# Mehooz/vision4leg

Measured on AMD Instinct MI355X. Metric: PPO env-steps/s (encoder+update, sim excluded), higher is better.
Workload: dtype f16; 1 GPU; ppo_locotransformer thin-goal: LocoTransformer S=93 A=6, E=32 envs x T=512, B=1024, 3 opt epochs; net=loco, envs_per_gpu=32, horizon=512, minibatch=1024, opt_epochs=3, parallelism=dp1, includes_rollout_inference=True, logp_old=recorded at action time (target_pf forward skipped; SURVEY 8d declared saving)

## Files before the change

### vision4leg_amd/csrc/gemm.h

```cpp
#pragma once
#include "common.h"

namespace v4l {

struct RowCtx {
  int64_t base;
  int a, b;
  int valid;
};

__device__ __forceinline__ void zero8(float (&v)[8]) {
#pragma unroll
  for (int j = 0; j < 8; ++j) v[j] = 0.f;
}
__device__ __forceinline__ void ld8(const float* p, float (&v)[8]) {
  const float4 x = *reinterpret_cast<const float4*>(p);
  const float4 y = *reinterpret_cast<const float4*>(p + 4);
  v[0] = x.x; v[1] = x.y; v[2] = x.z; v[3] = x.w;
  v[4] = y.x; v[5] = y.y; v[6] = y.z; v[7] = y.w;
}
template <typename H>
__device__ __forceinline__ void ld8(const H* p, float (&v)[8]) {
  static_assert(sizeof(H) == 2, "16-bit operand type");
  typedef typename HVec<H, 4>::type bf16x4;
  const bf16x4 x = *reinterpret_cast<const bf16x4*>(p);
  const bf16x4 y = *reinterpret_cast<const bf16x4*>(p + 4);
#pragma unroll
  for (int j = 0; j < 4; ++j) { v[j] = (float)x[j]; v[4 + j] = (float)y[j]; }
}

template <int W> __device__ __forceinline__ void ldv(const float* p, float (&v)[W]) {
  if constexpr (W == 1) v[0] = p[0];
  else if constexpr (W == 2) { const float2 x = *reinterpret_cast<const float2*>(p); v[0] = x.x; v[1] = x.y; }
  else { const float4 x = *reinterpret_cast<const float4*>(p); v[0] = x.x; v[1] = x.y; v[2] = x.z; v[3] = x.w; }
}
template <int W, typename H> __device__ __forceinline__ void ldv(const H* p, float (&v)[W]) {
  static_assert(sizeof(H) == 2, "16-bit operand type");
  if constexpr (W == 1) v[0] = (float)p[0];
  else {
    typedef typename HVec<H, W>::type bv_t;
    const bv_t x = *reinterpret_cast<const bv_t*>(p);
#pragma unroll
    for (int i = 0; i < W; ++i) v[i] = (float)x[i];
  }
}

__device__ __forceinline__ void keep8(float (&v)[8], bool ok) {
#pragma unroll
  for (int j = 0; j < 8; ++j) v[j] = ok ? v[j] : 0.f;
}

struct ADense {
  const float* p;
  int lda, M, K;
  const int* rowidx;
  int tokmap;
  const float* mask;
  __device__ __forceinline__ RowCtx row(int m) const {
    RowCtx rc;
    rc.valid = m < M;
    rc.a = rc.b = 0;
    int r = m;
    if (tokmap == 1) r = (m >> 4) * 17 + 1 + (m & 15);
    if (rowidx != nullptr) r = rowidx[rc.valid ? m : 0];
    rc.base = (int64_t)r * lda;
    return rc;
  }
  __device__ __forceinline__ void load(const RowCtx& rc, int k0, float (&v)[8]) const {
    const bool ok = rc.valid && k0 < K;
    const int64_t off = ok ? rc.base + k0 : 0;
    ld8(p + off, v);
    if (mask != nullptr) {
      float mk[8];
      ld8(mask + off, mk);
#pragma unroll
      for (int j = 0; j < 8; ++j) v[j] = mk[j] > 0.f ? v[j] : 0.f;
    }
    keep8(v, ok);
  }
  struct RowIt { int m; };
  __device__ __forceinline__ RowIt iter(int m) const { return RowIt{m}; }
  __device__ __forceinline__ int64_t off(const RowIt& it, int& valid) const { return row_off(it.m, valid); }
  __device__ __forceinline__ void next(RowIt& it) const { ++it.m; }
  __device__ __forceinline__ int64_t row_off(int m, int& valid) const { RowCtx rc = row(m); valid = rc.valid; return rc.base; }
  __device__ __forceinline__ int64_t col_off(int k, int& valid) const { valid = k < K; return k; }
  __device__ __forceinline__ float get(int64_t off) const {
    const float v = p[off];
    if (mask == nullptr) return v;
    const float mk = mask[off];
// ... 543 lines not shown

  float* out = slab + (int64_t)bz * Npad * Kpad;
#pragma unroll
  for (int i = 0; i < NT; ++i) {
    const int n = n0 + i * 16 + (lane & 15);
#pragma unroll
    for (int j = 0; j < KT; ++j) {
      const int k4 = k0 + (wave * KT + j) * 16 + (lane >> 4) * 4;
      if (n < Npad && k4 < Kpad)
        *reinterpret_cast<float4*>(out + (int64_t)n * Kpad + k4) = float4{acc[i][j][0], acc[i][j][1], acc[i][j][2], acc[i][j][3]};
    }
  }
  if (do_bias) {
    sBias[wave][lane] = bsum;
    __syncthreads();
    if (tid < BN && n0 + tid < Npad)
      bslab[(int64_t)bz * Npad + n0 + tid] = sBias[0][tid] + sBias[1][tid] + sBias[2][tid] + sBias[3][tid];
  }
}

template <typename T, int BN, int KT, class YL, class XL>
__global__ __launch_bounds__(256) void gemm_tn_kernel(YL yl, XL xl, int M, int m_per_block, float* __restrict__ slab,
                                                      float* __restrict__ bslab, int Npad, int Kpad) {
  tn_body<T, BN, KT, YL, XL>(yl, xl, M, m_per_block, slab, bslab, Npad, Kpad, blockIdx.x, blockIdx.y, blockIdx.z);
}

struct TnProb {
  ADense y, x;
  int M, mpb, Npad, Kpad, gx, gy;
  float* slab;
  float* bslab;
  int64_t blk0;
};
struct ADenseG {
  const V4L_GLOBAL float* p;
  const V4L_GLOBAL int* rowidx;
  const V4L_GLOBAL float* mask;
  int lda, M, K, tokmap;
  __device__ __forceinline__ explicit ADenseG(const ADense& a)
      : p(as_global(a.p)), rowidx(as_global(a.rowidx)), mask(as_global(a.mask)), lda(a.lda), M(a.M), K(a.K), tokmap(a.tokmap) {}
  struct RowIt { int m; };
  __device__ __forceinline__ RowIt iter(int m) const { return RowIt{m}; }
  __device__ __forceinline__ void next(RowIt& it) const { ++it.m; }
  __device__ __forceinline__ int64_t off(const RowIt& it, int& valid) const {
    const int m = it.m;
    valid = m < M;
    int r = m;
    if (tokmap == 1) r = (m >> 4) * 17 + 1 + (m & 15);
    if (a_rowidx()) r = rowidx[valid ? m : 0];
    return (int64_t)r * lda;
  }
  __device__ __forceinline__ bool a_rowidx() const { return rowidx != nullptr; }
  __device__ __forceinline__ int64_t col_off(int k, int& valid) const { valid = k < K; return k; }
  __device__ __forceinline__ float get(int64_t o) const {
    const float v = p[o];
    if (mask == nullptr) return v;
    const float mk = mask[o];
    return mk > 0.f ? v : 0.f;
  }
  template <int W> __device__ __forceinline__ void getv(int64_t o, float (&v)[W]) const {
#pragma unroll
    for (int i = 0; i < W; ++i) v[i] = get(o + i);
  }
};
template <typename T>
__global__ __launch_bounds__(256) void gemm_tn_group_kernel(const TnProb* __restrict__ probs, int np) {
  const TnProb p = probs[find_desc(probs, np, (int64_t)blockIdx.x)];
  const int lb = (int)((int64_t)blockIdx.x - p.blk0);
  const int bx = lb % p.gx, t = lb / p.gx;
  tn_body<T, 64, 1, ADenseG, ADenseG>(ADenseG(p.y), ADenseG(p.x), p.M, p.mpb, p.slab, p.bslab, p.Npad, p.Kpad, bx, t % p.gy,
                                      t / p.gy);
}

struct TnWide {
  const void *y, *x;
  int M, mpb, N, K;
  float *slab, *bslab;
  int blk0, pad;
};
template <typename T> struct Pair;
template <> struct Pair<__bf16> { typedef __attribute__((ext_vector_type(2))) __bf16 type; };
template <> struct Pair<_Float16> { typedef __attribute__((ext_vector_type(2))) _Float16 type; };
template <> struct Pair<float> { typedef __attribute__((ext_vector_type(2))) float type; };
template <typename H>
__device__ __forceinline__ void st8raw(H* dst, const H (&v)[8]) {
  static_assert(sizeof(H) == 2, "16-bit operand type");
  typename Frag<H>::type t;
#pragma unroll
  for (int j = 0; j < 8; ++j) t[j] = v[j];
  *reinterpret_cast<typename Frag<H>::type*>(dst) = t;
}
__device__ __forceinline__ void st8raw(float* dst, const float (&v)[8]) {
  *reinterpret_cast<float4*>(dst) = float4{v[0], v[1], v[2], v[3]};
  *reinterpret_cast<float4*>(dst + 4) = float4{v[4], v[5], v[6], v[7]};
}
template <typename T> struct TnWideLds {
  static constexpr int LD = 64 + (sizeof(T) == 2 ? 8 : 4);
  static constexpr size_t bytes(int N, int K) { return (size_t)(N + K) * LD * sizeof(T) + (size_t)8 * N * 4; }
  static constexpr size_t max_bytes = (size_t)(256 + 64) * LD * sizeof(T) + (size_t)8 * 256 * 4;
};

template <typename T, int N, int K>
__device__ __forceinline__ void tn_wide_body(const TnWide& p, int bz, unsigned char* smem) {
  constexpr int LD = TnWideLds<T>::LD;
  constexpr int NC = N / 64, KC = K / 64;
  constexpr bool SPLIT_N = N > 64;
  static_assert(!SPLIT_N || K == 64, "tn_wide: unsupported shape");
  constexpr int NT_W = SPLIT_N ? N / 64 : 4;
  constexpr int KT_W = SPLIT_N ? 4 : K / 64;
  typedef typename Frag<T>::type frag_t;
  typedef typename Pair<T>::type pair_t;
  T* sY = reinterpret_cast<T*>(smem);
  T* sX = sY + N * LD;
  float* sB = reinterpret_cast<float*>(sX + K * LD);
  const int tid = threadIdx.x, lane = tid & 63, wave = tid >> 6;
  const int half = lane >> 5, cl = (lane & 31) * 2;
  const int mb = bz * p.mpb, me = min(p.M, mb + p.mpb);
  const V4L_GLOBAL T* Y = as_global(reinterpret_cast<const T*>(p.y));
  const V4L_GLOBAL T* X = as_global(reinterpret_cast<const T*>(p.x));
  typedef const V4L_GLOBAL pair_t* gpair_t;
  pair_t yv[NC][8], xv[KC][8];
  float bs[NC][2];
#pragma unroll
  for (int q = 0; q < NC; ++q) bs[q][0] = bs[q][1] = 0.f;
  auto gload = [&](int ms) {
    const int r0 = ms + wave * 16 + half * 8;
#pragma unroll
    for (int j = 0; j < 8; ++j) {
// ... 82 lines not shown
    for (int k = 0; k < 8; ++k) t += sB[k * N + tid];
    as_global(p.bslab)[(int64_t)bz * N + tid] = t;
  }
}

template <typename T>
__global__ __launch_bounds__(256) void gemm_tn_wide_kernel(const TnWide* __restrict__ probs, int np) {
  extern __shared__ __attribute__((aligned(16))) unsigned char tn_wide_smem[];
  int pi = 0;
  for (int i = 1; i < np; ++i) pi = probs[i].blk0 <= (int)blockIdx.x ? i : pi;
  const TnWide p = probs[pi];
  const int bz = (int)blockIdx.x - p.blk0;
  if (p.N == 256 && p.K == 64) tn_wide_body<T, 256, 64>(p, bz, tn_wide_smem);
  else if (p.N == 192 && p.K == 64) tn_wide_body<T, 192, 64>(p, bz, tn_wide_smem);
  else if (p.N == 64 && p.K == 256) tn_wide_body<T, 64, 256>(p, bz, tn_wide_smem);
  else tn_wide_body<T, 64, 64>(p, bz, tn_wide_smem);
}
template <typename T>
__global__ __launch_bounds__(256) void gemm_tn_dense_kernel(const TnWide* __restrict__ wprobs, int nw, int wblocks,
                                                            const TnProb* __restrict__ gprobs, int ng) {
  extern __shared__ __attribute__((aligned(16))) unsigned char tn_wide_smem[];
  if ((int)blockIdx.x < wblocks) {
    int pi = 0;
    for (int i = 1; i < nw; ++i) pi = wprobs[i].blk0 <= (int)blockIdx.x ? i : pi;
    const TnWide p = wprobs[pi];
    const int bz = (int)blockIdx.x - p.blk0;
    if (p.N == 256 && p.K == 64) tn_wide_body<T, 256, 64>(p, bz, tn_wide_smem);
    else if (p.N == 192 && p.K == 64) tn_wide_body<T, 192, 64>(p, bz, tn_wide_smem);
    else if (p.N == 64 && p.K == 256) tn_wide_body<T, 64, 256>(p, bz, tn_wide_smem);
    else tn_wide_body<T, 64, 64>(p, bz, tn_wide_smem);
  } else {
    const int64_t b = (int64_t)blockIdx.x - wblocks;
    const TnProb p = gprobs[find_desc(gprobs, ng, b)];
    const int lb = (int)(b - p.blk0);
    const int bx = lb % p.gx, t = lb / p.gx;
    tn_body<T, 64, 1, ADenseG, ADenseG, true>(ADenseG(p.y), ADenseG(p.x), p.M, p.mpb, p.slab, p.bslab, p.Npad, p.Kpad, bx,
                                              t % p.gy, t / p.gy, tn_wide_smem);
  }
}
static inline bool tn_wide_shape(int N, int K) {
  return (N == 256 && K == 64) || (N == 192 && K == 64) || (N == 64 && K == 256) || (N == 64 && K == 64);
}

constexpr int CONV_BWD_MAX_BLOCKS = 256;

struct RedDesc {
  const float* slab;
  const float* bslab;
  float* dW;
  float* db;
  int nsplit, N, K, Npad, Kpad, Ktorch, Cin, taps;
  int64_t blk0;
  int group, pad_;
};
__global__ __launch_bounds__(256) void wgrad_reduce_kernel(const RedDesc* __restrict__ descs, int nd, float* __restrict__ sq_part,
                                                           int blk_base, float unscale) {
  __shared__ float part[4][64];
  const int64_t bid = (int64_t)blockIdx.x + blk_base;
  const RedDesc d = descs[find_desc(descs, nd, bid)];
  const int o = threadIdx.x & 63, g = threadIdx.x >> 6;
  const int64_t e = (bid - d.blk0) * 64 + o;
  const int64_t nk = (int64_t)d.N * d.K;
  const V4L_GLOBAL float* p = nullptr;
  int64_t stride = 0;
  int n = 0, k = 0;
  if (e < nk) {
    n = (int)(e / d.K); k = (int)(e - (int64_t)n * d.K);
    p = as_global(d.slab) + (int64_t)n * d.Kpad + k;
    stride = (int64_t)d.Npad * d.Kpad;
  } else if (d.db != nullptr && e < nk + d.N) {
// ... 33 lines not shown
```

### vision4leg_amd/csrc/net.h

```cpp
#pragma once
#include <string>
#include <vector>

#include "../../include/v4l_hip.h"
#include "elem.h"
#include "gemm.h"

namespace v4l { struct RowsChain; struct FbLoss; }

namespace v4l {

struct ParamInfo {
  std::string name;
  int ndim;
  int64_t shape[4];
  int64_t numel;
  int64_t goff;
};

struct Lin {
  int w = -1, b = -1;
  int N = 0, K = 0;
  int Np = 0, Kp = 0;
  int64_t pk = 0;
// ... 42 lines not shown
  std::vector<int64_t> deh;
  std::vector<LayerBw> lb;
  std::vector<int64_t> dxl;
  int64_t dhc = 0;
  int64_t dpool = 0, dc3 = 0, dc2 = 0, dc1 = 0;
  std::vector<int64_t> wps_wg, wps_tk;
  int64_t slab = 0;
  int64_t total = 0;
};

enum class LayerFamily {
  NONE,
  WPS_PLAIN,
  WPS_VIS,
  WPS_VIS17,
  WPS_OPT,
  WPS_OPT_VIS,
  BLOCK_STACK,
  BLOCK_PER_LAYER,
  LAYER_BY_LAYER,
};
struct LayerRoute {
  LayerFamily family = LayerFamily::NONE;
  bool heads_in = false;
  bool tail_in = false;
  bool rows17 = false;
  bool fb_allowed = false;
  bool heads_ext_allowed = false;
  bool heads_ext_critic = false;
  bool taps = false;
  bool stack_ok = true;
  bool tok0_in = false;
  int par_wgrad = 2;
  bool wps() const { return family >= LayerFamily::WPS_PLAIN && family <= LayerFamily::WPS_OPT_VIS; }
  bool opt() const { return family == LayerFamily::WPS_OPT || family == LayerFamily::WPS_OPT_VIS; }
  bool block() const { return family == LayerFamily::BLOCK_STACK || family == LayerFamily::BLOCK_PER_LAYER; }
};

}

struct v4l_net {
  v4l_net_cfg cfg;
  int Sp = 0;
  int ntok = v4l::NTOK;
  bool want_acts16 = false;
  const float* acts16_c1 = nullptr;
  bool vis_only() const { return cfg.kind == V4L_NET_CNN_VIS || cfg.kind == V4L_NET_LOCO_VIS; }
  bool is_tf() const { return cfg.kind == V4L_NET_LOCO || cfg.kind == V4L_NET_LOCO_VIS; }
  std::vector<v4l::ParamInfo> params;
  int64_t total_params = 0;
  v4l::Conv conv[3];
  v4l::Lin upconv, proj;
  std::vector<v4l::Lin> enc;
  std::vector<v4l::TLayer> layers;
  v4l::LNp fin_ln;
  v4l::LNp tok_ln, stok_ln;
  std::vector<v4l::Lin> head;
  int logstd = -1;
  int64_t packed_elems = 0;
  std::vector<v4l::PackDesc> packs;
  std::vector<int> pack_param;
  int64_t pack_blocks = 0;
  std::vector<float*> p;
  void* packed = nullptr;
  v4l::PackDesc* d_packs = nullptr;
  v4l::ParamSeg* d_segs = nullptr;
// ... 84 lines not shown
```

### vision4leg_amd/csrc/v4l_hip.hip

```cpp
#include <math.h>
#include <stdarg.h>

#include <algorithm>
#include <type_traits>

#include <dlfcn.h>

#include "net.h"
#include "infer.h"
#include "bwd.h"
#include "wps.h"
#include "wps_fb.h"
#include "rollout_dense.h"
#include "dense_stack.h"
#include "host_step.h"

namespace v4l {

static thread_local char g_err[1024] = "";
static bool sw_on(const char* name) { return getenv(name) != nullptr; }
template <typename T> struct TypeTag { typedef T type; };
#ifdef V4L_DEV_ONLY
template <class F> static inline int by_compute(int compute, F&& f) {
  typedef std::conditional<V4L_DEV_ONLY == V4L_BF16, __bf16, std::conditional<V4L_DEV_ONLY == V4L_F16, _Float16, float>::type>::type T;
// ... 267 lines not shown
    V4L_REQUIRE(net->tnp.size() <= (size_t)v4l_net::MAX_TNP, "internal: too many deferred weight-grads");
    for (TnProb& q : net->tnp) { const int64_t nb = q.blk0; q.blk0 = gb; gb += nb; }
    const size_t bytes = net->tnp.size() * sizeof(TnProb);
    if (net->tnp_cached.size() != net->tnp.size() || memcmp(net->tnp_cached.data(), net->tnp.data(), bytes) != 0) {
      V4L_REQUIRE(!capturing(c.s), "internal: weight-grad geometry changed while capturing a graph");
      V4L_HIP_CHECK(hipStreamSynchronize(c.s));
      V4L_HIP_CHECK(hipMemcpy(net->d_tnp, net->tnp.data(), bytes, hipMemcpyHostToDevice));
      net->tnp_cached = net->tnp;
    }
  }
  if (!net->wide.empty()) {
    V4L_REQUIRE(net->wide.size() <= (size_t)v4l_net::MAX_WIDE, "internal: too many fused-layer weight-grads");
    for (TnWide& q : net->wide) { const int nb = q.blk0; q.blk0 = wb; wb += nb; }
    const size_t bytes = net->wide.size() * sizeof(TnWide);
    if (net->wide_cached.size() != net->wide.size() || memcmp(net->wide_cached.data(), net->wide.data(), bytes) != 0) {
      V4L_REQUIRE(!capturing(c.s), "internal: weight-grad geometry changed while capturing a graph");
      V4L_HIP_CHECK(hipStreamSynchronize(c.s));
      V4L_HIP_CHECK(hipMemcpy(net->d_wide, net->wide.data(), bytes, hipMemcpyHostToDevice));
      net->wide_cached = net->wide;
    }
  }
  constexpr size_t dense_lds = TnWideLds<T>::max_bytes > TnBodyLds<T, 64, 1>::bytes ? TnWideLds<T>::max_bytes : TnBodyLds<T, 64, 1>::bytes;
  V4L_HIP_CHECK(lds_limit<&gemm_tn_wide_kernel<T>>(TnWideLds<T>::max_bytes));
  V4L_HIP_CHECK(lds_limit<&gemm_tn_dense_kernel<T>>(dense_lds));
  if (gb > 0 && wb > 0) {
    g_op = "layer.wgrad";
    V4L_KLAUNCH("gemm_tn_dense", net->wide_flops + net->tnp_flops, dg, gemm_tn_dense_kernel<T>, dim3((unsigned)(wb + gb)), dim3(256),
                dense_lds, dg, (const TnWide*)net->d_wide, (int)net->wide.size(), wb, (const TnProb*)net->d_tnp, (int)net->tnp.size());
    V4L_LAUNCH_CHECK();
    return 0;
  }
  if (gb > 0) {
    g_op = "dense.wgrad";
    V4L_KLAUNCH("gemm_tn_group", net->tnp_flops, dg, gemm_tn_group_kernel<T>, dim3((unsigned)gb), dim3(256), 0, dg,
                (const TnProb*)net->d_tnp, (int)net->tnp.size());
    V4L_LAUNCH_CHECK();
  }
  if (wb > 0) {
    g_op = "layer.wgrad";
    V4L_KLAUNCH("gemm_tn_wide", net->wide_flops, dg, gemm_tn_wide_kernel<T>, dim3((unsigned)wb), dim3(256),
                TnWideLds<T>::max_bytes, dg, (const TnWide*)net->d_wide, (int)net->wide.size());
    V4L_LAUNCH_CHECK();
  }
  return 0;
}
static int wgrad_reduce_prepare(Ctx& c, int64_t (&blocks)[2]) {
  v4l_net* net = c.net;
  std::stable_partition(net->red.begin(), net->red.end(), [](const RedDesc& d) { return d.group == 1; });
  int64_t blk = 0;
  blocks[0] = blocks[1] = 0;
  for (RedDesc& d : net->red) {
    d.blk0 = blk;
    const int64_t nb = cdiv64((int64_t)d.N * d.K + d.N, 64);
    blk += nb;
    blocks[d.group == 1 ? 0 : 1] += nb;
  }
  V4L_REQUIRE(net->red.size() <= (size_t)v4l_net::MAX_RED, "internal: too many weight-grad descriptors");
  const size_t bytes = net->red.size() * sizeof(RedDesc);
  if (net->red_cached.size() != net->red.size() || memcmp(net->red_cached.data(), net->red.data(), bytes) != 0) {
    V4L_REQUIRE(!capturing(c.s), "internal: weight-grad geometry changed while capturing a graph");
    V4L_HIP_CHECK(hipStreamSynchronize(c.s));
    if (c.tn != c.s) V4L_HIP_CHECK(hipStreamSynchronize(c.tn));
    V4L_HIP_CHECK(hipMemcpy(net->d_red, net->red.data(), bytes, hipMemcpyHostToDevice));
    net->red_cached = net->red;
  }
  float* sq = blk <= net->sq_cap() ? net->d_sq : nullptr;
  net->red_blocks = sq != nullptr ? (int)blk : 0;
  net->red_grads = c.grads;
// ... 645 lines not shown
  return 0;
}

int64_t v4l_net::table_bytes() const {
  return (int64_t)(packs.size() * sizeof(PackDesc) + params.size() * sizeof(ParamSeg) + MAX_RED * sizeof(RedDesc) +
                   MAX_TNP * sizeof(TnProb) + MAX_WIDE * sizeof(TnWide) + sq_cap() * sizeof(float) + 1024);
}
static bool dense_stack_shape(const v4l_net* N) {
  const v4l_net_cfg& c = N->cfg;
  if (sw_on("V4L_NO_DENSE_STACK")) return false;
  if (c.n_head_hidden != 2 || c.head_hidden[0] != 256 || c.head_hidden[1] != 256 || c.out_dim > OUT_LD) return false;
  for (int i = 0; i < 3; ++i)
    if (N->head[i].pkf < 0 || N->head[i].pkft < 0) return false;
  if (c.kind == V4L_NET_CNN_VIS) return N->head[0].Kp == 1024 && N->head[0].Rt == 1024;
  if (c.kind != V4L_NET_CNN) return false;
  return c.visual_dim == 256 && c.n_enc_hidden == 2 && c.enc_hidden[0] == 256 && c.enc_hidden[1] == 256 && N->proj.pkf >= 0 &&
         N->proj.pkft >= 0 && N->proj.Kp == 1024 && N->enc[1].pkft >= 0 && N->head[0].Kp == 512;
}
static bool mlp_256(const v4l_net_cfg& c) {
  return c.n_enc_hidden == 2 && c.enc_hidden[0] == 256 && c.enc_hidden[1] == 256 && c.state_dim <= 128;
}
static bool head_256(const v4l_net_cfg& c) { return c.n_head_hidden == 2 && c.head_hidden[0] == 256 && c.head_hidden[1] == 256; }
static bool depth_64(const v4l_net_cfg& c) { return c.in_channels == 4 && c.img_hw == 64; }
bool v4l_net::wps_tail_shape() const {
  return cfg.n_enc_hidden == 2 && cfg.enc_hidden[0] == 256 && cfg.enc_hidden[1] == 256;
}
LayerRoute v4l_net::layer_route(bool whole_pass) const {
  const v4l_net_cfg& c = cfg;
  LayerRoute r;
  r.taps = sw_on("V4L_LAYER_TAPS");
  r.stack_ok = !sw_on("V4L_NO_LAYER_STACK");
  r.tok0_in = sw_on("V4L_WPS_TOK0_IN");
  r.par_wgrad = sw_int("V4L_PAR_WGRAD", 2);
  const bool no_wps = sw_on("V4L_NO_WPS_LAYERS"), vis17 = sw_on("V4L_VIS17"), no_fb = sw_on("V4L_NO_FB");
  const bool head_in = sw_on("V4L_WPS_HEAD_IN"), ext_critic = sw_on("V4L_WPS_HEAD_EXT_CRITIC");
  if (!is_tf()) return r;
  const bool vis = c.kind == V4L_NET_LOCO_VIS, opt = c.token_norm || c.pytorch_encoder;
  const bool heads = head_256(c) && c.out_dim <= OUT_LD;
  const bool wps = c.ff_dim == 256 && c.n_layers == 2 && heads && layers[0].inproj.pkp >= 0 && !no_wps &&
                   (!vis || head[0].pko >= 0);
  const bool around = wps && whole_pass && !c.max_pool && r.stack_ok && !r.taps;
  r.family = LayerFamily::LAYER_BY_LAYER;
  if (vis) {
    if (wps && whole_pass && !opt) r.family = (vis17 || r.taps) ? LayerFamily::WPS_VIS17 : LayerFamily::WPS_VIS;
    else if (around && opt) r.family = LayerFamily::WPS_OPT_VIS;
    r.rows17 = r.wps();
    r.heads_in = r.wps() && !c.pytorch_encoder;
    r.tail_in = r.wps() && !c.token_norm;
    return r;
  }
  const bool plain = !opt && wps_tail_shape();
  if (wps && plain && r.stack_ok) {
    r.family = LayerFamily::WPS_PLAIN;
    r.heads_in = r.tail_in = true;
    r.heads_ext_allowed = !head_in && !r.taps;
    r.heads_ext_critic = r.heads_ext_allowed && ext_critic;
    r.fb_allowed = r.heads_ext_allowed && !c.max_pool && !no_fb && !ext_critic && c.out_dim <= ACT_CAP_NARROW;
  } else if (around && !plain) {
    r.family = LayerFamily::WPS_OPT;
    r.heads_in = !c.pytorch_encoder;
    r.tail_in = !c.token_norm && wps_tail_shape();
  } else if (c.ff_dim == 256 && !opt) {
    r.heads_in = c.n_layers >= 1 && heads && !c.max_pool;
    r.tail_in = c.n_layers >= 1 && wps_tail_shape();
    r.family = (r.heads_in && c.n_layers == 2 && r.stack_ok) ? LayerFamily::BLOCK_STACK : LayerFamily::BLOCK_PER_LAYER;
  }
// ... 589 lines not shown
    float* hand = ws + L.dhc;
    Epi din = mk_epi(hand, cw, cw);
    if ((rc = chain_bwd<T>(cx, head.data(), nh + 1, dense(ws + L.vis, cw, n, cw), hacts, dy, dhhp, &din))) return rc;
    {
      ADense yv = dense(hand, cw, n, c.visual_dim, nullptr, 0, ws + L.vis);
      if ((rc = lin_wgrad<T>(cx, proj, yv, dense(ws + L.c3, 1024, n, 1024), 1024))) return rc;
      Epi ep = mk_epi(ws + L.dc3, 1024, 1024);
      ep.mask = ws + L.c3;
      ep.ldmask = 1024;
      if ((rc = lin_dgrad<T>(cx, proj, yv, ep))) return rc;
    }
    {
      ADense ys = dense(hand + c.visual_dim, cw, n, c.enc_hidden[ne - 1], nullptr, 0, ws + L.vis + c.visual_dim);
      if ((rc = chain_bwd<T>(cx, enc.data(), ne, sin, eacts, ys, dehp, nullptr))) return rc;
    }
    return conv_bwd_and_wgrads();
  }

  if (c.kind == V4L_NET_CNN_VIS) {
    Epi din = mk_epi(ws + L.dc3, 1024, 1024);
    din.mask = ws + L.c3;
    din.ldmask = 1024;
    if ((rc = chain_bwd<T>(cx, head.data(), nh + 1, dense(ws + L.c3, 1024, n, 1024), hacts, dy, dhhp, &din))) return rc;
    return conv_bwd_and_wgrads();
  }

  const bool vis = c.kind == V4L_NET_LOCO_VIS;
  const int pw = vis ? TD : 2 * TD;
  const bool vis_opt = r.family == LayerFamily::WPS_OPT_VIS;
  const int R = n * (vis_opt ? NTOK : ntok);
  auto zero_row0 = [&](float* rows) {
    return hipMemset2DAsync(rows, (size_t)NTOK * TD * sizeof(float), 0, (size_t)TD * sizeof(float), (size_t)n, s);
  };
  if (r.heads_in) {
    if ((rc = lin_wgrad<T>(cx, head[2], dy, dense(hacts[1].p, 256, n, 256), 256))) return rc;
    if ((rc = lin_wgrad<T>(cx, head[1], dense(dhhp[1], 256, n, 256), dense(hacts[0].p, 256, n, 256), 256))) return rc;
    if (r.rows17) rc = lin_wgrad<T>(cx, head[0], dense(dhhp[0], 256, n, 256), dense(ws + L.pooled + TD, 2 * TD, n, TD), TD);
    else rc = lin_wgrad<T>(cx, head[0], dense(dhhp[0], 256, n, 256), dense(ws + L.pooled, 2 * TD, n, 2 * TD), 2 * TD);
    if (rc) return rc;
  } else {
    Epi din = mk_epi(ws + L.dpool, pw, pw);
    if ((rc = chain_bwd<T>(cx, head.data(), nh + 1, dense(ws + L.pooled, pw, n, pw), hacts, dy, dhhp, &din)))
      return rc;
    g_op = "pool";
    float* dlast = c.pytorch_encoder ? ws + L.dxfin : ws + L.dxl[c.n_layers];
    const float* xlast = c.pytorch_encoder ? ws + L.xfin : ws + L.x[c.n_layers];
    if (vis_opt) V4L_HIP_CHECK(zero_row0(dlast));
    if (vis)
      V4L_KLAUNCH("pool_bwd", 0, s, pool_all_bwd_kernel, dim3(n), dim3(64), 0, s, ws + L.dpool, n, ntok, vis_opt ? NTOK : ntok,
                  dlast + (vis_opt ? TD : 0), xlast + (vis_opt ? TD : 0), c.max_pool);
    else
      V4L_KLAUNCH("pool_bwd", 0, s, pool_bwd_kernel, dim3(n), dim3(64), 0, s, ws + L.dpool, n, dlast, xlast, c.max_pool);
    V4L_LAUNCH_CHECK();
    if (c.pytorch_encoder) {
      g_op = "final_ln";
      if ((rc = ln_bwd_launch(cx, std::min(cdiv(R, 16), 128), dlast, ws + L.dxl[c.n_layers], ws + L.xhF, ws + L.rsF, fin_ln, R))) return rc;
    }
  }
  const int lnb = std::min(cdiv(R, 16), 128);
  auto reduce_ln_partials = [&](const TLayer& t, const float* part, int nblk) {
    const int lnp[4] = {t.ln2.g, t.ln2.b, t.ln1.g, t.ln1.b};
    for (int q = 0; q < 4; ++q) {
      RedDesc o;
      memset(&o, 0, sizeof(o));
      o.slab = part + (int64_t)q * nblk * TD;
      o.dW = grads + params[lnp[q]].goff;
      o.nsplit = nblk; o.N = 1; o.K = TD; o.Npad = 1; o.Kpad = TD; o.Ktorch = TD;
      red.push_back(o);
    }
  };
  const bool stacked = r.family == LayerFamily::BLOCK_STACK && r.tail_in;
  if (r.wps()) {
// ... 35 lines not shown
      bt.wpt = base + proj.pkt; bt.wf2t = base + enc[1].pkt;
      bt.s_e1 = eacts[1].p; bt.s_e0 = eacts[0].p; bt.o_dhc = ws + L.dhc; bt.o_de0 = dehp[0];
    }
    WpsTailExtra tx;
    tx.wupt_f = base + upconv.pkpt;
    tx.dpool = ws + L.dpool;
    tx.xlast = c.max_pool ? ws + L.x[c.n_layers] : nullptr;
    tx.dyrows = !r.heads_in ? ws + L.dxl[c.n_layers] : nullptr;
    g_op = "layer";
    const double fl_heads = 2.0 * n * 2 * (16 * 256 + 256 * 256 + 256 * 128) / 2, fl_tok0 = 2.0 * n * (64 * 256 + 256 * 256);
    const double fl = 2 * 4.0 * n * 872576.0 + (head_ext ? 0.0 : 2 * fl_heads) + (tok0_ext ? 0.0 : fl_tok0) + 2.0 * n * 16 * 64 * 64;
#define V4L_WPS_BWD(TAPS_, VIS_, HIN_, TIN_, MODE_)                                                                       \
  do {                                                                                                                    \
    V4L_HIP_CHECK(lds_limit<&wps_layer_bwd_kernel<T, 2, TAPS_, VIS_, HIN_, TIN_, MODE_>>(WpsBwdLds<T>::bytes));            \
    V4L_KLAUNCH("wps_layer_bwd_stack", fl, s, (wps_layer_bwd_kernel<T, 2, TAPS_, VIS_, HIN_, TIN_, MODE_>), dim3(nblk), dim3(256), \
                (WpsBwdLds<T>::bytes), s, d, bh, bt, tx, n);                                                              \
  } while (0)
    const FbLoss* fbl = fb_loss;
    fb_loss = nullptr;
    V4L_REQUIRE(fbl == nullptr || (r.fb_allowed && !head_ext),
                "internal: a fused forward-loss-backward pass was prepared for a net that does not take it");
    const bool m_out = r.opt() && !r.tail_in, m_in = r.opt() && !r.heads_in;
    if (fbl != nullptr) {
      InfLayerStack fst;
      memset(&fst, 0, sizeof(fst));
      fst.nl = 2;
      for (int k = 0; k < 2; ++k)
        fst.l[k].n[0] = inf_layer<T>(this, layers[k], true, k == 0 ? ws + L.x[0] : nullptr);
      InfHeadPair fhd;
      memset(&fhd, 0, sizeof(fhd));
      fhd.n[0] = inf_head<T>(this, L, ws, false);
      FbLoss lo = *fbl;
      lo.dout = ws + L.dout;
      cx.slab_used = (cx.slab_used + 1) & ~(int64_t)1;
      lo.part = reinterpret_cast<double*>(cx.slab + cx.slab_used);
      V4L_REQUIRE((reinterpret_cast<uintptr_t>(lo.part) & 7) == 0, "internal: partial-statistics block not 8-byte aligned");
      cx.slab_used += 2 * (int64_t)nblk * FB_PART;
      V4L_REQUIRE(cx.slab_used <= slab_cap, "internal: weight-grad slab arena overflow");
      const double fl_fb = fl + 2.0 * n * (2 * 872576.0 + 99840.0);
      V4L_HIP_CHECK(lds_limit<&wps_layer_fb_kernel<T, true>>(WpsFbLds<T>::bytes));
      V4L_HIP_CHECK(lds_limit<&wps_layer_fb_kernel<T, false>>(WpsFbLds<T>::bytes));
      if (tok0_ext)
        V4L_KLAUNCH("wps_layer_fb_stack", fl_fb, s, (wps_layer_fb_kernel<T, false>), dim3(nblk), dim3(256), (WpsFbLds<T>::bytes), s, fst,
                    fhd, d, bh, bt, tx, lo, n);
      else
        V4L_KLAUNCH("wps_layer_fb_stack", fl_fb, s, (wps_layer_fb_kernel<T, true>), dim3(nblk), dim3(256), (WpsFbLds<T>::bytes), s, fst,
                    fhd, d, bh, bt, tx, lo, n);
      cx.fb_pending = true;
      cx.fb_args = lo;
      cx.fb_blocks = nblk;
      cx.fb_n = n;
    } else
    switch (r.family) {
      case LayerFamily::WPS_OPT_VIS:
        if (m_out && m_in) V4L_WPS_BWD(false, 2, true, true, 3);
        else if (m_in) V4L_WPS_BWD(false, 2, true, true, 2);
        else V4L_WPS_BWD(false, 2, true, true, 1);
        break;
      case LayerFamily::WPS_OPT:
        if (m_out && m_in) V4L_WPS_BWD(false, false, true, true, 3);
        else if (m_in) V4L_WPS_BWD(false, false, true, true, 2);
        else V4L_WPS_BWD(false, false, true, true, 1);
        break;
      case LayerFamily::WPS_VIS17:
        if (taps) V4L_WPS_BWD(true, true, true, true, 0);
        else V4L_WPS_BWD(false, true, true, true, 0);
// ... 1754 lines not shown
```

### vision4leg_amd/csrc/wps_fb.h

```cpp
#pragma once
#include "wps.h"

#pragma clang fp contract(on)

namespace v4l {

enum { FBP_LP = 0, FBP_LP2, FBP_SUR, FBP_LPMAX, FBP_LPMIN, FBP_RMAX, FBP_RMIN, FBP_SAT, FBP_DL = 8, FBP_VF = 16, FB_PART = 24 };

struct FbLoss {
  int actor;
  const float *ret, *oldv;
  int clipped;
  float clip;
  ActorArgs aa;
  const int* rowidx;
  float inv_n, gscale;
  float* dout;
  double* part;
  float* st;
};

template <typename T> struct WpsFbLds {
  static constexpr bool LDSW = sizeof(T) == 2;
  static constexpr size_t f_b = WpsFwdLds<T>::main_b, b_b = WpsBwdLds<T>::main_b;
  static constexpr size_t main_b = f_b > b_b ? f_b : b_b;
  static constexpr size_t red_b = WpsBwdLds<T>::red_b;
  static constexpr size_t so_b = 16 * 16 * 4;
  static constexpr size_t rec_b = (size_t)WPS_WPB * FB_PART * 8;
  static constexpr size_t bytes = main_b + (size_t)WPS_P_TOTAL * 4 + red_b + so_b + rec_b;
  static_assert(bytes <= 160 * 1024, "one block per CU");
};

__device__ __forceinline__ ActorRow fb_actor_row(const ActorArgs& p, const ActorDims& D, const float (&mu)[8], int slot, float amean,
                                                 float astd) {
  ActorRow o;
  float lp = 0.f;
#pragma unroll
  for (int a = 0; a < 8; ++a) {
    if (a < p.A) {
      const float act = p.acts[(int64_t)slot * p.A + a];
      const float d = act - mu[a];
      const float var = D.sg[a] * D.sg[a];
      lp += -(d * d) / (2.f * var) - D.lsg[a] - HALF_LOG_2PI - 0.f;
      o.z2[a] = d * d / var;
      o.dm[a] = d / var;
    } else {
      o.z2[a] = 0.f; o.dm[a] = 0.f;
    }
  }
  const float lpo = p.logp_old[slot];
  const float ratio = expf(lp - lpo);
  const float an = (p.adv[slot] - amean) / (astd + 1e-5f);
// ... 73 lines not shown
#pragma unroll
    for (int mt = 0; mt < 2; ++mt)
#pragma unroll
      for (int nt = 0; nt < 4; ++nt) xr[mt][nt] = xo[mt][nt];
  }
  float4 mk0[4], mk1[4];
  {
    const InfHead& h = fhd.n[0];
    float* pooled = reinterpret_cast<float*>(smem);
    T* h1 = reinterpret_cast<T*>(pooled + 16 * LF::LDP);
    T* h2 = h1 + 16 * LF::LDF;
    float4 hb0[4], hb1[4];
    float hb2[4];
#pragma unroll
    for (int j = 0; j < 4; ++j) {
      hb0[j] = *reinterpret_cast<const float4*>(h.b0 + nt4[j] * 16 + qr);
      hb1[j] = *reinterpret_cast<const float4*>(h.b1 + nt4[j] * 16 + qr);
      hb2[j] = h.b2[min(qr + j, h.nout - 1)];
    }
    GemmRing<T, 4, 4> ring0 = gemm_prefetch<T, 4, 4>((const T*)h.w0, 128, nt4, lane);
    __syncthreads();
    for (int i = tid; i < 16 * LF::LDP; i += 256) pooled[i] = 0.f;
    __syncthreads();
#pragma unroll
    for (int nt = 0; nt < 4; ++nt) {
      const float4 m = fr == 0 ? xr[1][nt] : xr[0][nt];
      const float4 mv = float4{rowsum16(m.x) * (1.f / 16.f), rowsum16(m.y) * (1.f / 16.f), rowsum16(m.z) * (1.f / 16.f),
                               rowsum16(m.w) * (1.f / 16.f)};
      if (fr == 0 && live) {
        const float4 t0 = xr[0][nt];
        *reinterpret_cast<float4*>(pooled + wave * LF::LDP + nt * 16 + qr) = t0;
        *reinterpret_cast<float4*>(pooled + wave * LF::LDP + TD + nt * 16 + qr) = mv;
        if (h.s_pooled != nullptr) {
          *reinterpret_cast<float4*>(h.s_pooled + (int64_t)smp * 128 + nt * 16 + qr) = t0;
          *reinterpret_cast<float4*>(h.s_pooled + (int64_t)smp * 128 + TD + nt * 16 + qr) = mv;
        }
      }
    }
    __syncthreads();
    f32x4 acc[1][4];
    auto store_h = [&](T* dst, const float4 (&bias)[4], float* save, float4 (&mk)[4]) {
#pragma unroll
      for (int j = 0; j < 4; ++j) {
        const int n4 = nt4[j] * 16 + qr;
        const float4 bb = bias[j];
        const float v0 = fmaxf(acc[0][j][0] + bb.x, 0.f), v1 = fmaxf(acc[0][j][1] + bb.y, 0.f);
        const float v2 = fmaxf(acc[0][j][2] + bb.z, 0.f), v3 = fmaxf(acc[0][j][3] + bb.w, 0.f);
        mk[j] = float4{v0, v1, v2, v3};
        st4(dst + fr * LF::LDF + n4, v0, v1, v2, v3);
        if (fr < ns) st4(save + (int64_t)(s0 + fr) * 256 + n4, v0, v1, v2, v3);
      }
    };
    zero_acc(acc);
    block_gemm<T, 1, 4, 4>(acc, pooled, LF::LDP, (const T*)h.w0, 128, nt4, lane, ring0);
    GemmRing<T, 4, 8> ring1 = gemm_prefetch<T, 4, 8>((const T*)h.w1, 256, nt4, lane);
    store_h(h1, hb0, h.s_h0, mk0);
    __syncthreads();
    zero_acc(acc);
    block_gemm<T, 1, 4, 8>(acc, h1, LF::LDF, (const T*)h.w1, 256, nt4, lane, ring1);
    store_h(h2, hb1, h.s_h1, mk1);
    __syncthreads();
    if (wave == 0) {
      const int nt0[1] = {0};
      f32x4 a1[1][1];
      zero_acc(a1);
      block_gemm<T, 1, 1, 8>(a1, h2, LF::LDF, (const T*)h.w2, 256, nt0, lane);
      float ov[4];
#pragma unroll
      for (int r = 0; r < 4; ++r) {
        const int c = qr + r;
        ov[r] = c < h.nout ? a1[0][0][r] + hb2[r] : 0.f;
        if (fr < ns) h.out[(int64_t)(s0 + fr) * OUT_LD + c] = ov[r];
      }
      *reinterpret_cast<float4*>(so + fr * 16 + qr) = float4{ov[0], ov[1], ov[2], ov[3]};
    }
  }
  const int nt2[2] = {wave * 2, wave * 2 + 1};
  GemmRing<T, 4, 2> ring2 = gemm_prefetch<T, 4, 2>((const T*)hd.w2t, 64, nt4, lane);
  GemmRing<T, 4, 8> ringb1 = gemm_prefetch<T, 4, 8>((const T*)hd.w1t, 256, nt4, lane);
  float* dt = reinterpret_cast<float*>(smem);
  T* dh1 = reinterpret_cast<T*>(dt + 16 * LB::LDX);
  T* dh0 = dh1 + 16 * LB::LDF;
  float* dpool = reinterpret_cast<float*>(dh0 + 16 * LB::LDF);
// ... 330 lines not shown
```

Baseline: 411,300 env-steps/s.

## Store head activations in f16 and use dedicated grouped wgrad kernel reading them

The fused forward/backward kernel now saves pooled features and head hidden activations as 16-bit values instead of fp32 when running in f16 with the fused loss path. The head weight-gradient GEMMs mark those operands as 16-bit and read them directly. A new tn_group_body replaces the generic tn_body path for grouped weight-gradient problems, with wave-level row index broadcast, paired column loads and LDS staging. The aim is to halve activation write and read traffic and to streamline the wgrad GEMM. In exchange, saved activations lose precision, and the launch now needs dynamic LDS.

```diff
diff --git a/vision4leg_amd/csrc/gemm.h b/vision4leg_amd/csrc/gemm.h
--- a/vision4leg_amd/csrc/gemm.h
+++ b/vision4leg_amd/csrc/gemm.h
@@ -55,6 +55,7 @@
   int lda, M, K;
   const int* rowidx;
   int tokmap;
+  int t16;
   const float* mask;
   __device__ __forceinline__ RowCtx row(int m) const {
     RowCtx rc;
@@ -664,52 +665,6 @@
   float* bslab;
   int64_t blk0;
 };
-struct ADenseG {
-  const V4L_GLOBAL float* p;
-  const V4L_GLOBAL int* rowidx;
-  const V4L_GLOBAL float* mask;
-  int lda, M, K, tokmap;
-  __device__ __forceinline__ explicit ADenseG(const ADense& a)
-      : p(as_global(a.p)), rowidx(as_global(a.rowidx)), mask(as_global(a.mask)), lda(a.lda), M(a.M), K(a.K), tokmap(a.tokmap) {}
-  struct RowIt { int m; };
-  __device__ __forceinline__ RowIt iter(int m) const { return RowIt{m}; }
-  __device__ __forceinline__ void next(RowIt& it) const { ++it.m; }
-  __device__ __forceinline__ int64_t off(const RowIt& it, int& valid) const {
-    const int m = it.m;
-    valid = m < M;
-    int r = m;
-    if (tokmap == 1) r = (m >> 4) * 17 + 1 + (m & 15);
-    if (a_rowidx()) r = rowidx[valid ? m : 0];
-    return (int64_t)r * lda;
-  }
-  __device__ __forceinline__ bool a_rowidx() const { return rowidx != nullptr; }
-  __device__ __forceinline__ int64_t col_off(int k, int& valid) const { valid = k < K; return k; }
-  __device__ __forceinline__ float get(int64_t o) const {
-    const float v = p[o];
-    if (mask == nullptr) return v;
-    const float mk = mask[o];
-    return mk > 0.f ? v : 0.f;
-  }
-  template <int W> __device__ __forceinline__ void getv(int64_t o, float (&v)[W]) const {
-#pragma unroll
-    for (int i = 0; i < W; ++i) v[i] = get(o + i);
-  }
-};
-template <typename T>
-__global__ __launch_bounds__(256) void gemm_tn_group_kernel(const TnProb* __restrict__ probs, int np) {
-  const TnProb p = probs[find_desc(probs, np, (int64_t)blockIdx.x)];
-  const int lb = (int)((int64_t)blockIdx.x - p.blk0);
-  const int bx = lb % p.gx, t = lb / p.gx;
-  tn_body<T, 64, 1, ADenseG, ADenseG>(ADenseG(p.y), ADenseG(p.x), p.M, p.mpb, p.slab, p.bslab, p.Npad, p.Kpad, bx, t % p.gy,
-                                      t / p.gy);
-}
-
-struct TnWide {
-  const void *y, *x;
-  int M, mpb, N, K;
-  float *slab, *bslab;
-  int blk0, pad;
-};
 template <typename T> struct Pair;
 template <> struct Pair<__bf16> { typedef __attribute__((ext_vector_type(2))) __bf16 type; };
 template <> struct Pair<_Float16> { typedef __attribute__((ext_vector_type(2))) _Float16 type; };
@@ -726,6 +681,188 @@
   *reinterpret_cast<float4*>(dst) = float4{v[0], v[1], v[2], v[3]};
   *reinterpret_cast<float4*>(dst + 4) = float4{v[4], v[5], v[6], v[7]};
 }
+template <typename T>
+__device__ __forceinline__ void tn_group_body(const TnProb& p, int bx, int by, int bz, unsigned char* smem) {
+  constexpr int BN = 64, BMR = 64, NT = BN / 16;
+  constexpr int LD = BMR + (sizeof(T) == 2 ? 8 : 4);
+  typedef typename Frag<T>::type frag_t;
+  typedef typename Pair<T>::type pair_t;
+  typedef Pair<float>::type fpair_t;
+  T* sY = reinterpret_cast<T*>(smem);
+  T* sX = sY + BN * LD;
+  float (*sBias)[64] = reinterpret_cast<float (*)[64]>(sX + 64 * LD);
+  const int tid = threadIdx.x, lane = tid & 63;
+  const int wave = __builtin_amdgcn_readfirstlane(tid >> 6);
+  const int k0 = bx * 64, n0 = by * BN;
+  const int mb = bz * p.mpb;
+  const int me = min(p.M, mb + p.mpb);
+  const int mey = min(me, p.y.M), mex = min(me, p.x.M);
+  const bool do_bias = (p.bslab != nullptr) && (bx == 0);
+  const V4L_GLOBAL float* Yp = as_global(p.y.p);
+  const V4L_GLOBAL float* Ym = as_global(p.y.mask);
+  const V4L_GLOBAL int* Yr = as_global(p.y.rowidx);
+  const V4L_GLOBAL float* Xp = as_global(p.x.p);
+  const V4L_GLOBAL float* Xm = as_global(p.x.mask);
+  const V4L_GLOBAL int* Xr = as_global(p.x.rowidx);
+  const int ylda = p.y.lda, xlda = p.x.lda;
+  const bool ytok = p.y.tokmap == 1, xtok = p.x.tokmap == 1;
+  const bool x16 = sizeof(T) == 2 && p.x.t16 != 0;
+  const bool yok = n0 + lane < p.y.K;
+  const int yco = yok ? n0 + lane : 0;
+  const int xhalf = lane >> 5, xcl = (lane & 31) * 2;
+  const bool xok = k0 + xcl < p.x.K;
+  const int xco = xok ? k0 + xcl : 0;
+
+  float yv[16];
+  fpair_t xf[8];
+  pair_t xp[8];
+  float bsum = 0.f;
+  auto gload = [&](int ms) {
+    const int ry0 = ms + wave * 16;
+    int rr;
+    {
+      const int rv = ry0 + (lane & 15);
+      rr = ytok ? rv + (rv >> 4) + 1 : rv;
+      if (Yr != nullptr) rr = Yr[rv < mey ? rv : 0];
+#pragma unroll
+      for (int j = 0; j < 16; ++j) {
+        const int r = __builtin_amdgcn_readlane(rr, j);
+        const int64_t ro = ry0 + j < mey ? (int64_t)r * ylda : 0;
+        yv[j] = Yp[ro + yco];
+      }
+    }
+    const int rx0 = ms + wave * 16 + xhalf * 8;
+    int64_t xo[8];
+    if (Xr != nullptr) {
+#pragma unroll
+      for (int j = 0; j < 8; ++j) xo[j] = (int64_t)Xr[rx0 + j < mex ? rx0 + j : 0];
+    } else {
+#pragma unroll
+      for (int j = 0; j < 8; ++j) { const int m = rx0 + j; xo[j] = xtok ? m + (m >> 4) + 1 : m; }
+    }
+#pragma unroll
+    for (int j = 0; j < 8; ++j) xo[j] = (rx0 + j < mex ? xo[j] * xlda : 0) + xco;
+    if (x16) {
+      if constexpr (sizeof(T) == 2) {
+        const V4L_GLOBAL T* X16 = reinterpret_cast<const V4L_GLOBAL T*>(Xp);
+#pragma unroll
+        for (int j = 0; j < 8; ++j) xp[j] = *reinterpret_cast<const V4L_GLOBAL pair_t*>(X16 + xo[j]);
+      }
+    } else {
+#pragma unroll
+      for (int j = 0; j < 8; ++j) xf[j] = *reinterpret_cast<const V4L_GLOBAL fpair_t*>(Xp + xo[j]);
+      if (Xm != nullptr) {
+#pragma unroll
+        for (int j = 0; j < 8; ++j) {
+          const fpair_t mk = *reinterpret_cast<const V4L_GLOBAL fpair_t*>(Xm + xo[j]);
+          xf[j].x = mk.x > 0.f ? xf[j].x : 0.f;
+          xf[j].y = mk.y > 0.f ? xf[j].y : 0.f;
+        }
+      }
+    }
+    if (Ym != nullptr) {
+#pragma unroll
+      for (int j = 0; j < 16; ++j) {
+        const int r = __builtin_amdgcn_readlane(rr, j);
+        const int64_t ro = ry0 + j < mey ? (int64_t)r * ylda : 0;
+        const float mk = Ym[ro + yco];
+        yv[j] = mk > 0.f ? yv[j] : 0.f;
+      }
+    }
+  };
+  auto lstore = [&](int ms) {
+    const int ry0 = ms + wave * 16, rx0 = ry0 + xhalf * 8;
+#pragma unroll
+    for (int g = 0; g < 2; ++g) {
+      float t8[8];
+#pragma unroll
+      for (int j = 0; j < 8; ++j) {
+        t8[j] = (yok && ry0 + g * 8 + j < mey) ? yv[g * 8 + j] : 0.f;
+        bsum += t8[j];
+      }
+      st8<T>(&sY[lane * LD + wave * 16 + g * 8], t8);
+    }
+    T* d0 = &sX[xcl * LD + wave * 16 + xhalf * 8];
+    if (x16) {
+      if constexpr (sizeof(T) == 2) {
+        T c0[8], c1[8];
+#pragma unroll
+        for (int j = 0; j < 8; ++j) {
+          const bool ok = xok && rx0 + j < mex;
+          c0[j] = ok ? xp[j].x : (T)0.f;
+          c1[j] = ok ? xp[j].y : (T)0.f;
+        }
+        st8raw(d0, c0);
+        st8raw(d0 + LD, c1);
+      }
+    } else {
+      float c0[8], c1[8];
+#pragma unroll
+      for (int j = 0; j < 8; ++j) {
+        const bool ok = xok && rx0 + j < mex;
+        c0[j] = ok ? xf[j].x : 0.f;
+        c1[j] = ok ? xf[j].y : 0.f;
+      }
+      st8<T>(d0, c0);
+      st8<T>(d0 + LD, c1);
+    }
+  };
+
+  f32x4 acc[NT];
+#pragma unroll
+  for (int i = 0; i < NT; ++i) acc[i] = f32x4{0.f, 0.f, 0.f, 0.f};
+  const int fr = lane & 15, fg = (lane >> 4) * 8;
+#pragma unroll 1
+  for (int ms = mb; ms < me; ms += BMR) {
+    gload(ms);
+    lstore(ms);
+    __syncthreads();
+#pragma unroll
+    for (int ks = 0; ks < BMR / 32; ++ks) {
+      const frag_t fx = *reinterpret_cast<const frag_t*>(&sX[(wave * 16 + fr) * LD + ks * 32 + fg]);
+#pragma unroll
+      for (int i = 0; i < NT; ++i) {
+        const frag_t fy = *reinterpret_cast<const frag_t*>(&sY[(i * 16 + fr) * LD + ks * 32 + fg]);
+        mma_k32(acc[i], fx, fy);
+      }
+    }
+    __syncthreads();
+  }
+
+  float* out = p.slab + (int64_t)bz * p.Npad * p.Kpad;
+#pragma unroll
+  for (int i = 0; i < NT; ++i) {
+    const int n = n0 + i * 16 + (lane & 15);
+    const int k4 = k0 + wave * 16 + (lane >> 4) * 4;
+    if (n < p.Npad && k4 < p.Kpad)
+      *reinterpret_cast<float4*>(out + (int64_t)n * p.Kpad + k4) = float4{acc[i][0], acc[i][1], acc[i][2], acc[i][3]};
+  }
+  if (do_bias) {
+    sBias[wave][lane] = bsum;
+    __syncthreads();
+    if (tid < BN && n0 + tid < p.Npad)
+      p.bslab[(int64_t)bz * p.Npad + n0 + tid] = sBias[0][tid] + sBias[1][tid] + sBias[2][tid] + sBias[3][tid];
+  }
+}
+template <typename T>
+__device__ __forceinline__ void tn_group_block(const TnProb& p, int64_t b, unsigned char* smem) {
+  const int lb = (int)(b - p.blk0);
+  const int bx = lb % p.gx, t = lb / p.gx;
+  tn_group_body<T>(p, bx, t % p.gy, t / p.gy, smem);
+}
+template <typename T>
+__global__ __launch_bounds__(256) void gemm_tn_group_kernel(const TnProb* __restrict__ probs, int np) {
+  extern __shared__ __attribute__((aligned(16))) unsigned char tn_group_smem[];
+  const TnProb p = probs[find_desc(probs, np, (int64_t)blockIdx.x)];
+  tn_group_block<T>(p, (int64_t)blockIdx.x, tn_group_smem);
+}
+
+struct TnWide {
+  const void *y, *x;
+  int M, mpb, N, K;
+  float *slab, *bslab;
+  int blk0, pad;
+};
 template <typename T> struct TnWideLds {
   static constexpr int LD = 64 + (sizeof(T) == 2 ? 8 : 4);
   static constexpr size_t bytes(int N, int K) { return (size_t)(N + K) * LD * sizeof(T) + (size_t)8 * N * 4; }
@@ -874,10 +1011,7 @@
   } else {
     const int64_t b = (int64_t)blockIdx.x - wblocks;
     const TnProb p = gprobs[find_desc(gprobs, ng, b)];
-    const int lb = (int)(b - p.blk0);
-    const int bx = lb % p.gx, t = lb / p.gx;
-    tn_body<T, 64, 1, ADenseG, ADenseG, true>(ADenseG(p.y), ADenseG(p.x), p.M, p.mpb, p.slab, p.bslab, p.Npad, p.Kpad, bx,
-                                              t % p.gy, t / p.gy, tn_wide_smem);
+    tn_group_block<T>(p, b, tn_wide_smem);
   }
 }
 static inline bool tn_wide_shape(int N, int K) {
diff --git a/vision4leg_amd/csrc/net.h b/vision4leg_amd/csrc/net.h
--- a/vision4leg_amd/csrc/net.h
+++ b/vision4leg_amd/csrc/net.h
@@ -98,6 +98,7 @@
   bool stack_ok = true;
   bool tok0_in = false;
   int par_wgrad = 2;
+  bool wgrad_ops_f32 = false;
   bool wps() const { return family >= LayerFamily::WPS_PLAIN && family <= LayerFamily::WPS_OPT_VIS; }
   bool opt() const { return family == LayerFamily::WPS_OPT || family == LayerFamily::WPS_OPT_VIS; }
   bool block() const { return family == LayerFamily::BLOCK_STACK || family == LayerFamily::BLOCK_PER_LAYER; }
diff --git a/vision4leg_amd/csrc/v4l_hip.hip b/vision4leg_amd/csrc/v4l_hip.hip
--- a/vision4leg_amd/csrc/v4l_hip.hip
+++ b/vision4leg_amd/csrc/v4l_hip.hip
@@ -323,8 +323,8 @@
   }
   if (gb > 0) {
     g_op = "dense.wgrad";
-    V4L_KLAUNCH("gemm_tn_group", net->tnp_flops, dg, gemm_tn_group_kernel<T>, dim3((unsigned)gb), dim3(256), 0, dg,
-                (const TnProb*)net->d_tnp, (int)net->tnp.size());
+    V4L_KLAUNCH("gemm_tn_group", net->tnp_flops, dg, gemm_tn_group_kernel<T>, dim3((unsigned)gb), dim3(256),
+                (TnBodyLds<T, 64, 1>::bytes), dg, (const TnProb*)net->d_tnp, (int)net->tnp.size());
     V4L_LAUNCH_CHECK();
   }
   if (wb > 0) {
@@ -1036,6 +1036,7 @@
   r.stack_ok = !sw_on("V4L_NO_LAYER_STACK");
   r.tok0_in = sw_on("V4L_WPS_TOK0_IN");
   r.par_wgrad = sw_int("V4L_PAR_WGRAD", 2);
+  r.wgrad_ops_f32 = sw_on("V4L_WGRAD_OPS_F32");
   const bool no_wps = sw_on("V4L_NO_WPS_LAYERS"), vis17 = sw_on("V4L_VIS17"), no_fb = sw_on("V4L_NO_FB");
   const bool head_in = sw_on("V4L_WPS_HEAD_IN"), ext_critic = sw_on("V4L_WPS_HEAD_EXT_CRITIC");
   if (!is_tf()) return r;
@@ -1691,12 +1692,14 @@
   auto zero_row0 = [&](float* rows) {
     return hipMemset2DAsync(rows, (size_t)NTOK * TD * sizeof(float), 0, (size_t)TD * sizeof(float), (size_t)n, s);
   };
+  const bool ops16 = sizeof(T) == 2 && fb_loss != nullptr && r.fb_allowed && !r.rows17 && !r.wgrad_ops_f32;
   if (r.heads_in) {
-    if ((rc = lin_wgrad<T>(cx, head[2], dy, dense(hacts[1].p, 256, n, 256), 256))) return rc;
-    if ((rc = lin_wgrad<T>(cx, head[1], dense(dhhp[1], 256, n, 256), dense(hacts[0].p, 256, n, 256), 256))) return rc;
-    if (r.rows17) rc = lin_wgrad<T>(cx, head[0], dense(dhhp[0], 256, n, 256), dense(ws + L.pooled + TD, 2 * TD, n, TD), TD);
-    else rc = lin_wgrad<T>(cx, head[0], dense(dhhp[0], 256, n, 256), dense(ws + L.pooled, 2 * TD, n, 2 * TD), 2 * TD);
-    if (rc) return rc;
+    ADense xh1 = dense(hacts[1].p, 256, n, 256), xh0 = dense(hacts[0].p, 256, n, 256);
+    ADense xpool = r.rows17 ? dense(ws + L.pooled + TD, 2 * TD, n, TD) : dense(ws + L.pooled, 2 * TD, n, 2 * TD);
+    xh1.t16 = xh0.t16 = xpool.t16 = ops16 ? 1 : 0;
+    if ((rc = lin_wgrad<T>(cx, head[2], dy, xh1, 256))) return rc;
+    if ((rc = lin_wgrad<T>(cx, head[1], dense(dhhp[1], 256, n, 256), xh0, 256))) return rc;
+    if ((rc = lin_wgrad<T>(cx, head[0], dense(dhhp[0], 256, n, 256), xpool, xpool.K))) return rc;
   } else {
     Epi din = mk_epi(ws + L.dpool, pw, pw);
     if ((rc = chain_bwd<T>(cx, head.data(), nh + 1, dense(ws + L.pooled, pw, n, pw), hacts, dy, dhhp, &din)))
@@ -1798,6 +1801,7 @@
       fhd.n[0] = inf_head<T>(this, L, ws, false);
       FbLoss lo = *fbl;
       lo.dout = ws + L.dout;
+      lo.ops16 = ops16 ? 1 : 0;
       cx.slab_used = (cx.slab_used + 1) & ~(int64_t)1;
       lo.part = reinterpret_cast<double*>(cx.slab + cx.slab_used);
       V4L_REQUIRE((reinterpret_cast<uintptr_t>(lo.part) & 7) == 0, "internal: partial-statistics block not 8-byte aligned");
diff --git a/vision4leg_amd/csrc/wps_fb.h b/vision4leg_amd/csrc/wps_fb.h
--- a/vision4leg_amd/csrc/wps_fb.h
+++ b/vision4leg_amd/csrc/wps_fb.h
@@ -18,6 +18,7 @@
   float* dout;
   double* part;
   float* st;
+  int ops16;
 };
 
 template <typename T> struct WpsFbLds {
@@ -157,8 +158,14 @@
         *reinterpret_cast<float4*>(pooled + wave * LF::LDP + nt * 16 + qr) = t0;
         *reinterpret_cast<float4*>(pooled + wave * LF::LDP + TD + nt * 16 + qr) = mv;
         if (h.s_pooled != nullptr) {
-          *reinterpret_cast<float4*>(h.s_pooled + (int64_t)smp * 128 + nt * 16 + qr) = t0;
-          *reinterpret_cast<float4*>(h.s_pooled + (int64_t)smp * 128 + TD + nt * 16 + qr) = mv;
+          if (sizeof(T) == 2 && lo.ops16) {
+            T* sp = reinterpret_cast<T*>(h.s_pooled) + (int64_t)smp * 128 + nt * 16 + qr;
+            st4(sp, t0.x, t0.y, t0.z, t0.w);
+            st4(sp + TD, mv.x, mv.y, mv.z, mv.w);
+          } else {
+            *reinterpret_cast<float4*>(h.s_pooled + (int64_t)smp * 128 + nt * 16 + qr) = t0;
+            *reinterpret_cast<float4*>(h.s_pooled + (int64_t)smp * 128 + TD + nt * 16 + qr) = mv;
+          }
         }
       }
     }
@@ -173,7 +180,10 @@
         const float v2 = fmaxf(acc[0][j][2] + bb.z, 0.f), v3 = fmaxf(acc[0][j][3] + bb.w, 0.f);
         mk[j] = float4{v0, v1, v2, v3};
         st4(dst + fr * LF::LDF + n4, v0, v1, v2, v3);
-        if (fr < ns) st4(save + (int64_t)(s0 + fr) * 256 + n4, v0, v1, v2, v3);
+        if (fr < ns) {
+          if (sizeof(T) == 2 && lo.ops16) st4(reinterpret_cast<T*>(save) + (int64_t)(s0 + fr) * 256 + n4, v0, v1, v2, v3);
+          else st4(save + (int64_t)(s0 + fr) * 256 + n4, v0, v1, v2, v3);
+        }
       }
     };
     zero_acc(acc);
```

New measurement: 410,600 env-steps/s. No clear change (-0.2%).
